# EvolvingLMMs-Lab/multimodal-sae

Measured on AMD Instinct MI355X. Metric: tokens/sec through SAE encode+TopK+decode, d=4096 width=131072, higher is better.
Workload: dtype int8 MFMA candidate select + f32 exact re-score/decode (outputs f32-exact); 1 GPU; BASELINE configs[1]: d_model=4096 width=131072 k=32, T=8192 bf16 activations/step resident in HBM, random-init unit-norm f32 weights; k=32, parallelism=single GPU, distinct_batches=4

## Files before the change

include/msae.h:

```cpp
#ifndef MSAE_H_
#define MSAE_H_

#include <stddef.h>
#include <stdint.h>

#ifdef __cplusplus
extern "C" {
#endif

#define MSAE_ABI_VERSION 4

enum { MSAE_F32 = 0, MSAE_BF16 = 1, MSAE_F16 = 2 };

enum {
  MSAE_EINVAL = -1,
  MSAE_EALIGN = -2,
  MSAE_EWS = -3,
  MSAE_ENOTIMPL = -4
};

enum { MSAE_COARSE_DEFAULT = -1, MSAE_COARSE_BF16 = 0, MSAE_COARSE_INT8 = 1, MSAE_COARSE_FP8 = 2 };
enum { MSAE_DITHER_DEFAULT = 0, MSAE_DITHER_ON = 1, MSAE_DITHER_OFF = 2 };
typedef struct msae_options {
  uint32_t size;
  int32_t coarse_mode;
  float guard_z;
  int32_t status_detail;
  void *profile;
  int32_t exact;
  int32_t dither;
  int32_t *rows_rescored;
  uint64_t dither_seed;
  int32_t certified;
  int32_t reserved2;
  const void *certified_operands;
} msae_options;
void msae_options_init(msae_options *opts);

int msae_abi_version(void);
const char *msae_error_string(int code);
const char *msae_target_arch(void);


int msae_pre_acts_f32(const void *x, int x_dtype, const float *W_enc, const float *b_enc,
                      const float *b_dec, int T, int d, int N, int relu, float *out, void *stream);

size_t msae_topk_ws_bytes(int T, int N, int k);
int msae_topk_f32(const float *latents, int T, int N, int k, float *vals, int32_t *idx, void *ws,
                  size_t ws_bytes, void *stream);


size_t msae_encoder_prepared_bytes(int N, int d);
int msae_encoder_prepare(const float *W_enc, int N, int d, void *prepared, void *stream);
int msae_encoder_prepare_opts(const float *W_enc, int N, int d, void *prepared, const msae_options *opts, void *stream);
size_t msae_encoder_certified_bytes(int N, int d);
int msae_encoder_prepare_certified(const float *W_enc, const float *b_enc, int N, int d, void *operands, void *stream);
int msae_encoder_refresh(const float *W_enc, int N, int d, void *prepared, const msae_options *opts,
                         void *stream);
int msae_encoder_refresh_for(const float *W_enc, int N, int d, void *prepared, int T_next, const msae_options *opts,
                             void *stream);

size_t msae_encode_topk_ws_bytes(int T, int d, int N, int k, const msae_options *opts);
int msae_encode_topk(const void *x, int x_dtype, const float *W_enc, const float *b_enc,
                     const float *b_dec, const void *prepared, int T, int d, int N, int k,
                     int set_feature, float set_value, int zero_feature, float *vals, int32_t *idx,
                     int32_t *status, void *ws, size_t ws_bytes, const msae_options *opts, void *stream);
int msae_encode_topk_i64(const void *x, int x_dtype, const float *W_enc, const float *b_enc,
                         const float *b_dec, const void *prepared, int T, int d, int N, int k,
                         int set_feature, float set_value, int zero_feature, float *vals, int64_t *idx,
                         int32_t *status, void *ws, size_t ws_bytes, const msae_options *opts, void *stream);

size_t msae_encode_topk_rows_ws_bytes(int max_rows, int N);
int msae_encode_topk_rows(const void *x, int x_dtype, const float *W_enc, const float *b_enc,
                          const float *b_dec, const int32_t *rows, const int32_t *n_rows, int max_rows,
                          int d, int N, int k, int set_feature, float set_value, int zero_feature,
                          float *vals, int64_t *idx, int32_t *status, void *ws, size_t ws_bytes, void *stream);

size_t msae_shard_record_bytes(int C);
int msae_shard_candidates(const void *x, int x_dtype, const float *b_enc_shard, const float *b_dec,
                          const void *prepared_shard, int T, int d, int N_shard, int k, int row_offset, int C,
                          int set_feature, int zero_feature, void *records, void *ws, size_t ws_bytes,
                          const msae_options *opts, void *stream);
size_t msae_rescore_candidates_ws_bytes(int T, int d, int N, int k, int G, int C);
int msae_rescore_candidates(const void *x, int x_dtype, const float *W_enc, const float *b_enc,
                            const float *b_dec, int T, int T_valid, int d, int N, int k, int G, int C,
                            const void *records, int set_feature, float set_value, int zero_feature,
                            float *vals, int64_t *idx, int32_t *status, void *ws, size_t ws_bytes,
                            const msae_options *opts, void *stream);


int msae_decode_f32(const int32_t *idx, const float *acts, const float *W_dec, const float *b_dec,
                    int A, int k, int N, int d, float *out, int32_t *status, void *stream);
int msae_decode_i64_f32(const int64_t *idx, const float *acts, const float *W_dec, const float *b_dec,
                        int A, int k, int N, int d, float *out, int32_t *status, void *stream);

int msae_decode_bwd_acts_f32(const int32_t *idx, const float *grad_out, const float *W_dec, int A,
                             int k, int N, int d, float *g_acts, int32_t *status, void *stream);

size_t msae_decode_bwd_wdec_ws_bytes(int A, int k, int N);
int msae_decode_bwd_wdec_f32(const int32_t *idx, const float *acts, const float *grad_out, int A,
                             int k, int N, int d, float *g_W_dec, float *row_sumsq, float *row_act_sum,
                             int32_t *status, void *ws, size_t ws_bytes, void *stream);

int msae_sparsify_count(const float *vals, const int32_t *idx, int B, int S, int k, float thresh,
                        const uint8_t *filter_bitmap, int N, int64_t *counts, void *stream);
int msae_sparsify_write(const float *vals, const int32_t *idx, int B, int S, int k, float thresh,
                        const uint8_t *filter_bitmap, int N, int64_t row_base,
                        const int64_t *counts, int64_t *locations, float *activations,
                        void *stream);

enum { MSAE_POOL_IMAGE = 0, MSAE_POOL_WINDOW = 1, MSAE_STATS_MAX_T = 65536 };
size_t msae_feature_stats_ws_bytes(int T, int k, int N);
int msae_feature_stats_update(const float *vals, const int32_t *idx, int B, int S, int k, float thresh, int N,
                              int mode, int pool_len, int window, int64_t row_base, int n_top, uint64_t *count,
                              float *act_max, double *act_sum, float *top_val, int64_t *top_id, void *ws,
                              size_t ws_bytes, void *stream);
int msae_feature_stats_merge(int N, int n_top, uint64_t *count, float *act_max, double *act_sum, float *top_val,
                             int64_t *top_id, const uint64_t *src_count, const float *src_max,
                             const double *src_sum, const float *src_val, const int64_t *src_id, void *stream);

typedef struct msae_feature_sample {
  uint32_t size;
  int32_t n_sample;
  uint64_t seed;
  uint64_t *seg_count;
  float *smp_val;
  int64_t *smp_id;
} msae_feature_sample;
int msae_feature_stats_update_sampled(const float *vals, const int32_t *idx, int B, int S, int k, float thresh, int N,
                                      int mode, int pool_len, int window, int64_t row_base, int n_top,
                                      uint64_t *count, float *act_max, double *act_sum, float *top_val,
                                      int64_t *top_id, const msae_feature_sample *sample, void *ws, size_t ws_bytes,
                                      void *stream);
int msae_feature_sample_merge(int N, int n_sample, uint64_t seed, uint64_t *seg_count, float *smp_val,
                              int64_t *smp_id, const uint64_t *src_seg_count, const float *src_val,
                              const int64_t *src_id, void *stream);

enum { MSAE_POOL_TOKEN = 2 };
enum { MSAE_COACT_JACCARD = 0, MSAE_COACT_COUNT = 1 };
size_t msae_coact_ws_bytes(int T, int k, int N);
int msae_coact_update(const float *vals, const int32_t *idx, int B, int S, int k, float thresh, int N, int mode,
                      int pool_len, int window, const int32_t *slot_of, int F, int32_t *counts, uint64_t *seg_count,
                      void *ws, size_t ws_bytes, void *stream);
int msae_coact_topk(const int32_t *counts, const int64_t *seg_count, const int32_t *queries, int F, int N, int m,
                    int metric, int exclude_self, float *out_val, int32_t *out_idx, void *stream);
int msae_coact_topk_i64(const int32_t *counts, const int64_t *seg_count, const int32_t *queries, int F, int N, int m,
                        int metric, int exclude_self, float *out_val, int64_t *out_idx, void *stream);

enum { MSAE_REDUCE_MEAN = 0, MSAE_REDUCE_MAX = 1, MSAE_PROBE_MAX_K = 256 };
int msae_pooled_acts_f32(const void *x, int x_dtype, const float *W_enc, const float *b_enc, const float *b_dec, int T,
                         int d, int N, const int32_t *seg, int S, const int32_t *chunks, int C, int reduce, float *out,
                         void *stream);
int msae_probe_maps_f32(const void *x, int x_dtype, const float *W_enc, const float *b_enc, const float *b_dec, int T,
                        int d, int N, const int32_t *seg, int S, const int32_t *idx, int k, float *maps, void *stream);

int msae_row_inv_norms_f32(const float *W, int N, int d, float *inv, void *stream);
size_t msae_rows_topk_ws_bytes(int M, int N, int k, int chunks);
int msae_rows_topk_f32(const float *Q, int Qn, const int32_t *q_rows, int M, const float *K, int N, int d,
                       const float *q_scale, const float *k_scale, const int32_t *exclude, int k, int chunks,
                       float *vals, int32_t *idx, void *ws, size_t ws_bytes, void *stream);
int msae_rows_topk_i64_f32(const float *Q, int Qn, const int32_t *q_rows, int M, const float *K, int N, int d,
                           const float *q_scale, const float *k_scale, const int32_t *exclude, int k, int chunks,
                           float *vals, int64_t *idx, void *ws, size_t ws_bytes, void *stream);

int msae_pre_acts_features_f32(const void *x, int x_dtype, const float *W_enc, const float *b_enc, const float *b_dec,
                               const int32_t *features, int M, int T, int d, int N, int relu,
                               float *out, int ld_out, void *stream);
int msae_topk_map_i64_f32(const float *latents, int T, int M, int k, int ld, const int32_t *col_map,
                          float *vals, int64_t *idx, void *stream);

enum { MSAE_EDIT_SET = 0, MSAE_EDIT_ZERO = 1 };
int msae_edit_topk_f32(const float *vals_in, const int32_t *idx_in, int T, int kk, const int32_t *edit_feat,
                       const float *edit_val, const int32_t *edit_kind, int E, int N, int k, float *vals, int32_t *idx,
                       void *stream);
int msae_edit_topk_i64_f32(const float *vals_in, const int64_t *idx_in, int T, int kk, const int32_t *edit_feat,
                           const float *edit_val, const int32_t *edit_kind, int E, int N, int k, float *vals,
                           int64_t *idx, void *stream);

int msae_edit_topk_rows_f32(const float *vals_in, const int32_t *idx_in, int T, int kk, const int32_t *group_of,
                            const int32_t *group_off, int G, const int32_t *edit_feat, const float *edit_val,
                            const int32_t *edit_kind, int E_total, int E_max, int N, int k, float *vals, int32_t *idx,
                            uint8_t *edited, void *stream);
int msae_edit_topk_rows_i64_f32(const float *vals_in, const int64_t *idx_in, int T, int kk, const int32_t *group_of,
                                const int32_t *group_off, int G, const int32_t *edit_feat, const float *edit_val,
                                const int32_t *edit_kind, int E_total, int E_max, int N, int k, float *vals, int64_t *idx,
                                uint8_t *edited, void *stream);

int msae_merge_topk(const int32_t *gathered, int T, int G, int kl, int k, float *vals, int32_t *idx,
                    int32_t *flagged, void *stream);
int msae_compact_flags(const int32_t *flags, int T, int32_t *rows, int32_t *n_rows, void *stream);
int msae_merge_topk_masked(const int32_t *gathered, int T, int G, int kl, int k, const int32_t *mask,
                           float *vals, int32_t *idx, int64_t *idx64, void *stream);

int msae_unit_norm_rows_f32(float *W, int N, int d, float eps, void *stream);
size_t msae_weighted_row_sum_ws_bytes(int N, int d);
int msae_weighted_row_sum_f32(const float *W, const float *s, int N, int d, float scale, float *out, void *ws,
                              size_t ws_bytes, void *stream);
int msae_sum_f32(const float *v, size_t n, float *accum, void *stream);
int msae_adam_rows_fused_f32(float *W, const float *G, float *M, float *V, int rows, int d,
                             const float *total_sumsq, float max_norm, int project, float lr, float beta1,
                             float beta2, float eps, int step, float renorm_eps, void *prepared, int T_next,
                             const msae_options *opts, void *stream);
int msae_grad_sumsq_f32(const float *g, size_t n, float *accum, void *stream);
int msae_adam_rows_f32(float *W, const float *G, float *M, float *V, int rows, int d,
                       const float *total_sumsq, float max_norm, int project, float lr, float beta1,
                       float beta2, float eps, int step, void *stream);

size_t msae_adam8_blocks(int rows, int d);
int msae_adam8_rows_f32(float *W, const float *G, uint8_t *M8, uint8_t *R8, float *SM, float *SR, int rows, int d,
                        const float *total_sumsq, float max_norm, int project, float lr, float beta1, float beta2,
                        float eps, int step, float renorm_eps, void *prepared, int T_next, const msae_options *opts,
                        void *stream);
int msae_adam8_quantize_f32(const float *M, const float *V, uint8_t *M8, uint8_t *R8, float *SM, float *SR, int rows,
                            int d, void *stream);
int msae_adam8_dequantize_f32(const uint8_t *M8, const uint8_t *R8, const float *SM, const float *SR, float *M, float *V,
                              int rows, int d, void *stream);

int msae_profile_create(int max_steps, void **handle);
int msae_profile_read(void *handle, float *stage_ms, int *n_steps);
int msae_profile_destroy(void *handle);

#ifdef __cplusplus
}
#endif
#endif
```

multimodal-sae_amd/csrc/capi.hip:

```cpp
#include "common.h"

extern "C" int msae_abi_version(void) { return MSAE_ABI_VERSION; }

extern "C" const char *msae_target_arch(void) { return "gfx950"; }

extern "C" const char *msae_error_string(int code) {
  switch (code) {
    case 0: return "success";
    case MSAE_EINVAL: return "msae: invalid argument (shape, k or dtype code)";
    case MSAE_EALIGN: return "msae: pointer or leading dimension not aligned as required";
    case MSAE_EWS: return "msae: workspace missing or too small";
    case MSAE_ENOTIMPL: return "msae: shape outside what this build supports";
    default: return code > 0 ? hipGetErrorString((hipError_t)code) : "msae: unknown error";
  }
}
```

multimodal-sae_amd/csrc/topk.hip:

```cpp
#include "common.h"
#include "sortsel.h"
#include "wave_ops.h"

namespace {

constexpr int TK_THREADS = 1024;
constexpr int TK_WAVES = TK_THREADS / 64;
constexpr int TK_BINS = 4096;

struct TkShared {
  unsigned hist[TK_BINS];
  unsigned wave_tot[TK_WAVES];
  unsigned bin;
  unsigned remaining;
  unsigned base_gt;
  unsigned base_eq;
};

template <bool VEC>
__device__ __forceinline__ void load4(const float *row, int i, int N, float (&v)[4]) {
  if constexpr (VEC) {
    f32x4 t = *reinterpret_cast<const f32x4 *>(row + i);
    v[0] = t[0]; v[1] = t[1]; v[2] = t[2]; v[3] = t[3];
  } else {
#pragma unroll
    for (int e = 0; e < 4; ++e) v[e] = (i + e < N) ? row[i + e] : 0.f;
  }
}

template <bool VEC>
__device__ __forceinline__ void radix_pass(const float *row, int N, unsigned prefix, unsigned mask,
                                           int shift, int nbins, TkShared &sh) {
  const unsigned need = sh.remaining;
  for (int b = threadIdx.x; b < nbins; b += TK_THREADS) sh.hist[b] = 0;
  __syncthreads();
  const int n4 = (N + 3) & ~3;
  for (int i = threadIdx.x * 4; i < n4; i += TK_THREADS * 4) {
    float v[4];
    load4<VEC>(row, i, N, v);
#pragma unroll
    for (int e = 0; e < 4; ++e) {
      if (VEC || i + e < N) {
        unsigned key = f32_order_key(v[e]);
        if ((key & mask) == prefix) atomicAdd(&sh.hist[(key >> shift) & (unsigned)(nbins - 1)], 1u);
      }
    }
  }
  __syncthreads();
  const int per = (nbins + TK_THREADS - 1) / TK_THREADS;
  const int rt = TK_THREADS - 1 - threadIdx.x;
  unsigned local = 0;
  for (int e = 0; e < per; ++e) {
    int b = nbins - 1 - (rt * per + e);
    if (b >= 0) local += sh.hist[b];
  }
  const int lane = threadIdx.x & 63, wave = threadIdx.x >> 6;
  unsigned incl = local;
#pragma unroll
  for (int off = 1; off < 64; off <<= 1) {
    unsigned n = __shfl_down(incl, off, 64);
    if (lane + off < 64) incl += n;
  }
  __syncthreads();
  if (lane == 0) sh.wave_tot[wave] = incl;
  __syncthreads();
  unsigned above = 0;
  for (int w = wave + 1; w < TK_WAVES; ++w) above += sh.wave_tot[w];
  above += incl - local;
  if (above < need && need <= above + local) {
    unsigned cum = above;
    for (int e = 0; e < per; ++e) {
      int b = nbins - 1 - (rt * per + e);
      if (b < 0) break;
      unsigned c = sh.hist[b];
      if (cum + c >= need) {
        sh.bin = (unsigned)b;
        sh.remaining = need - cum;
        break;
      }
      cum += c;
    }
  }
  __syncthreads();
}

template <bool VEC>
__global__ __launch_bounds__(TK_THREADS) void topk_rows_kernel(const float *__restrict__ latents,
                                                               int T, int N, int k, int ld,
                                                               const int *__restrict__ n_rows,
                                                               float *__restrict__ vals,
                                                               int32_t *__restrict__ idx, TopkExtra ex) {
  extern __shared__ __attribute__((aligned(16))) unsigned char smem_raw[];
  if (n_rows) T = min(T, *n_rows);
  TkShared &sh = *reinterpret_cast<TkShared *>(smem_raw);
  unsigned long long *keys = reinterpret_cast<unsigned long long *>(smem_raw + sizeof(TkShared));
  const int kp = next_pow2(k);
  for (int rowi = blockIdx.x; rowi < T; rowi += gridDim.x) {
  const float *row = latents + (size_t)rowi * ld;

  if (threadIdx.x == 0) {
    sh.remaining = (unsigned)k;
    sh.base_gt = 0;
    sh.base_eq = 0;
  }
  for (int i = threadIdx.x; i < kp; i += TK_THREADS) keys[i] = 0ull;
  __syncthreads();

  unsigned prefix = 0, mask = 0;
  radix_pass<VEC>(row, N, prefix, mask, 20, 4096, sh);
  prefix |= sh.bin << 20; mask |= 0xFFFu << 20;
  radix_pass<VEC>(row, N, prefix, mask, 8, 4096, sh);
  prefix |= sh.bin << 8; mask |= 0xFFFu << 8;
  radix_pass<VEC>(row, N, prefix, mask, 0, 256, sh);
  prefix |= sh.bin;
  const unsigned pivot = prefix;
  const unsigned r = sh.remaining;
  const unsigned n_gt = (unsigned)k - r;
  __syncthreads();

  const int n4 = (N + 3) & ~3;
  for (int base = 0; base < n4; base += TK_THREADS * 4) {
    const int i = base + threadIdx.x * 4;
    float v[4] = {0.f, 0.f, 0.f, 0.f};
    unsigned key[4];
    unsigned c_gt = 0, c_eq = 0;
    if (i < n4) load4<VEC>(row, i, N, v);
#pragma unroll
    for (int e = 0; e < 4; ++e) {
      const bool in = (i + e < N);
      key[e] = in ? f32_order_key(v[e]) : 0u;
      c_gt += (in && key[e] > pivot);
      c_eq += (in && key[e] == pivot);
    }
    const unsigned packed = c_gt | (c_eq << 16);
    if (__syncthreads_or((int)packed) == 0) continue;
    unsigned total;
    const unsigned ex = block_excl_scan<TK_WAVES>(packed, sh.wave_tot, &total);
    unsigned p_gt = sh.base_gt + (ex & 0xFFFFu);
    unsigned p_eq = sh.base_eq + (ex >> 16);
#pragma unroll
    for (int e = 0; e < 4; ++e) {
      if (i + e < N) {
        if (key[e] > pivot) {
          keys[p_gt++] = rank_key(v[e], i + e);
        } else if (key[e] == pivot) {
          if (p_eq < r) keys[n_gt + p_eq] = rank_key(v[e], i + e);
          ++p_eq;
        }
      }
    }
    __syncthreads();
    if (threadIdx.x == 0) {
      sh.base_gt += total & 0xFFFFu;
      sh.base_eq += total >> 16;
    }
    __syncthreads();
    if (sh.base_gt >= n_gt && sh.base_eq >= r) break;
  }
  __syncthreads();

  bitonic_sort_desc_u64<TK_THREADS>(keys, kp, threadIdx.x);
  const int orow = ex.row_map ? ex.row_map[rowi] : rowi;
  for (int j = threadIdx.x; j < k; j += TK_THREADS) {
    const unsigned long long kk = keys[j];
    const int ix = rank_key_index(kk);
    const int ox = ex.col_map ? ex.col_map[ix] : ix;
    if (idx) idx[(size_t)orow * k + j] = ox;
    if (ex.idx64) ex.idx64[(size_t)orow * k + j] = ox;
    vals[(size_t)orow * k + j] = row[ix];
  }
  if (ex.status && threadIdx.x == 0) ex.status[orow] = ex.detail ? (1 | ((ex.status[orow] & ~3) << 8)) : 1;
  __syncthreads();
  }
}

constexpr int KTH_LOW_BIT = 14;
template <int VPL>
__global__ __launch_bounds__(256) void kth_value_kernel(const float *__restrict__ rows, int T, int S,
                                                        int ld, int r, float *__restrict__ out,
                                                        int out_ld, int out_col, KthPush push) {
  const int lane = threadIdx.x & 63;
  const int t = blockIdx.x * 4 + (threadIdx.x >> 6);
  if (t >= T) return;
  const float *row = rows + (size_t)t * ld;
  unsigned key[VPL];
#pragma unroll
  for (int i = 0; i < VPL / 4; ++i) {
    const f32x4 v = *reinterpret_cast<const f32x4 *>(row + (i * 64 + lane) * 4);
    key[4 * i + 0] = f32_order_key(v[0]); key[4 * i + 1] = f32_order_key(v[1]);
    key[4 * i + 2] = f32_order_key(v[2]); key[4 * i + 3] = f32_order_key(v[3]);
  }
  unsigned lo = 0u;
  int first_bit = 31;
  {
    unsigned mx = 0u;
#pragma unroll
    for (int i = 0; i < VPL; ++i) mx = key[i] > mx ? key[i] : mx;
#pragma unroll
    for (int off = 32; off > 0; off >>= 1) { const unsigned o = __shfl_xor(mx, off, 64); mx = o > mx ? o : mx; }
    const unsigned pre = mx & 0xFF000000u;
    int c = 0;
#pragma unroll
    for (int i = 0; i < VPL; ++i) c += (key[i] >= pre) ? 1 : 0;
#pragma unroll
    for (int off = 32; off > 0; off >>= 1) c += __shfl_xor(c, off, 64);
    if (c >= r) { lo = pre; first_bit = 23; }
  }
#pragma unroll 1
  for (int bit = first_bit; bit >= KTH_LOW_BIT; --bit) {
    const unsigned mid = lo | (1u << bit);
    int c = 0;
#pragma unroll
    for (int i = 0; i < VPL; ++i) c += (key[i] >= mid) ? 1 : 0;
#pragma unroll
    for (int off = 32; off > 0; off >>= 1) c += __shfl_xor(c, off, 64);
    if (c >= r) lo = mid;
  }
  if (lane == 0) out[(size_t)t * out_ld + out_col] = f32_from_order_key(lo);
  if (push.cnt && f32_from_order_key(lo) > 0.f) {
    int total = 0;
#pragma unroll
    for (int i = 0; i < VPL; ++i) {
      total += __builtin_popcountll(__builtin_amdgcn_ballot_w64(key[i] > lo));
      if ((i & 7) == 7) asm volatile("" : "+s"(total));
    }
    if (total == 0) return;
    int base = 0;
    if (lane == 0) base = atomicAdd(push.cnt + (size_t)t * push.cnt_stride, total);
    base = __builtin_amdgcn_readfirstlane(base);
    unsigned long long *list = push.cand + (size_t)t * (push.row_stride ? push.row_stride : push.cap);
    unsigned lo2 = lo;
    asm volatile("" : "+v"(lo2));
#pragma unroll
    for (int i = 0; i < VPL; ++i) {
      const bool hit = key[i] > lo2;
      const unsigned long long m = __builtin_amdgcn_ballot_w64(hit);
      if (m == 0ull) continue;
      if (hit) {
        const int slot = base + (int)__builtin_amdgcn_mbcnt_hi((unsigned)(m >> 32), __builtin_amdgcn_mbcnt_lo((unsigned)m, 0u));
        const int j = ((i >> 2) * 64 + lane) * 4 + (i & 3);
        unsigned kk;
        asm volatile("v_mov_b32 %0, %1" : "=v"(kk) : "v"(key[i]));
        if (slot < push.cap) list[slot] = rank_key_from_order(kk, j * push.stride + push.off);
      }
      base += __builtin_popcountll(m);
      if ((i & 7) == 7) asm volatile("" : "+s"(base));
    }
  }
}

template <bool SECOND> struct MergeOut;
template <> struct MergeOut<false> { float *vals; int32_t *idx; int32_t *flagged; };
template <> struct MergeOut<true> { const int32_t *mask; float *vals; int32_t *idx; int64_t *idx64; };

template <bool SECOND>
__global__ __launch_bounds__(64) void merge_topk_kernel(const int32_t *__restrict__ gathered, int T, int G, int kl, int k,
                                                        MergeOut<SECOND> o) {
  extern __shared__ __attribute__((aligned(16))) unsigned long long mkeys[];
  const int lane = threadIdx.x, t = blockIdx.x;
  if constexpr (SECOND) { if (o.mask[t] == 0) return; }
  const int M = G * kl, np = next_pow2(M);
  unsigned long long worst_last = 0ull;
  for (int i = lane; i < np; i += 64) {
    unsigned long long key = 0ull;
    if (i < M) {
      const int g = i / kl, j = i % kl;
      const float v = __int_as_float(gathered[(((size_t)g * 2 + 0) * T + t) * kl + j]);
      const int f = gathered[(((size_t)g * 2 + 1) * T + t) * kl + j];
      key = rank_key(v, f);
      if constexpr (!SECOND) { if (j == kl - 1) worst_last = key > worst_last ? key : worst_last; }
    }
    mkeys[i] = key;
  }
  if constexpr (!SECOND) worst_last = wave_max(worst_last);
  bitonic_sort_desc_u64<64>(mkeys, np, lane);
  for (int j = lane; j < k; j += 64) {
    const unsigned long long key = mkeys[j];
    if constexpr (SECOND) {
      if (o.idx) o.idx[(size_t)t * k + j] = rank_key_index(key);
      if (o.idx64) o.idx64[(size_t)t * k + j] = rank_key_index(key);
    } else {
      o.idx[(size_t)t * k + j] = rank_key_index(key);
    }
    o.vals[(size_t)t * k + j] = rank_key_value(key);
  }
  if constexpr (!SECOND) { if (lane == 0 && o.flagged) o.flagged[t] = (kl < k && worst_last >= mkeys[k - 1]) ? 1 : 0; }
}

__global__ __launch_bounds__(1024) void compact_flags_kernel(const int32_t *__restrict__ flags, int T,
                                                             int32_t *__restrict__ rows, int32_t *__restrict__ n_rows) {
  __shared__ int wave_tot[16];
  const int lane = threadIdx.x & 63;
  int carry = 0;
  for (int base = 0; base < T; base += 1024) {
    const int t = base + threadIdx.x;
    const bool f = t < T && flags[t] != 0;
    const unsigned long long m = __builtin_amdgcn_ballot_w64(f);
    int total;
    const int off = carry + block_wave_offset<16>((int)__builtin_popcountll(m), wave_tot, &total);
    if (f) rows[off + __builtin_popcountll(m & ((1ull << lane) - 1ull))] = t;
    carry += total;
  }
  if (threadIdx.x == 0) *n_rows = carry;
}

}

extern "C" size_t msae_topk_ws_bytes(int T, int N, int k) {
  (void)T; (void)N; (void)k;
  return 0;
}

int msae_topk_launch(const float *latents, int T, int N, int k, int ld, const int *n_rows,
                     float *vals, int32_t *idx, hipStream_t s, const TopkExtra &ex) {
  if (T < 0 || N <= 0 || k <= 0 || k > N || k > 16384 || ld < N) return MSAE_EINVAL;
  if (T == 0) return 0;
  const size_t smem = sizeof(TkShared) + (size_t)next_pow2(k) * sizeof(unsigned long long);
  const bool vec = (N % 4 == 0) && (ld % 4 == 0) && msae_aligned(latents, 16);
  if (smem > 48 * 1024) {
    if (vec) MSAE_HIP_TRY(hipFuncSetAttribute((const void *)topk_rows_kernel<true>, hipFuncAttributeMaxDynamicSharedMemorySize, (int)smem));
    else MSAE_HIP_TRY(hipFuncSetAttribute((const void *)topk_rows_kernel<false>, hipFuncAttributeMaxDynamicSharedMemorySize, (int)smem));
  }
  const int grid = (n_rows && T > 128) ? 128 : T;
  if (vec)
    hipLaunchKernelGGL(topk_rows_kernel<true>, dim3(grid), dim3(TK_THREADS), smem, s, latents, T, N, k, ld,
                       n_rows, vals, idx, ex);
  else
    hipLaunchKernelGGL(topk_rows_kernel<false>, dim3(grid), dim3(TK_THREADS), smem, s, latents, T, N, k,
                       ld, n_rows, vals, idx, ex);
  return msae_launch_status();
}

bool msae_kth_value_launch(const float *rows, int T, int S, int ld, int r, float *out, int out_ld,
                           int out_col, hipStream_t s, const KthPush &push) {
  if (S % 256 || ld % 4 || !msae_aligned(rows, 16) || r < 1 || r > S) return false;
  const dim3 grid((T + 3) / 4), block(256);
  switch (S / 64) {
#define KTH_CASE(V) case V: hipLaunchKernelGGL(kth_value_kernel<V>, grid, block, 0, s, rows, T, S, ld, r, out, out_ld, out_col, push); return true;
    KTH_CASE(4) KTH_CASE(8) KTH_CASE(16) KTH_CASE(32) KTH_CASE(64) KTH_CASE(128)
#undef KTH_CASE
    default: return false;
  }
}

extern "C" int msae_topk_f32(const float *latents, int T, int N, int k, float *vals, int32_t *idx,
                             void *ws, size_t ws_bytes, void *stream) {
  (void)ws; (void)ws_bytes;
  return msae_topk_launch(latents, T, N, k, N, nullptr, vals, idx, (hipStream_t)stream, TopkExtra());
}

extern "C" int msae_topk_map_i64_f32(const float *latents, int T, int M, int k, int ld, const int32_t *col_map,
                                     float *vals, int64_t *idx, void *stream) {
  if (!latents || !col_map || !vals || !idx) return MSAE_EINVAL;
  TopkExtra ex;
  ex.idx64 = idx; ex.col_map = col_map;
  return msae_topk_launch(latents, T, M, k, ld, nullptr, vals, nullptr, (hipStream_t)stream, ex);
}

template <bool SECOND>
static int merge_topk_launch(const int32_t *gathered, int T, int G, int kl, int k, MergeOut<SECOND> o, void *stream) {
  if (T < 0 || G <= 0 || kl <= 0 || k <= 0 || (long)G * kl < k || (long)G * kl > 8192) return MSAE_EINVAL;
  if (T == 0) return 0;
  const size_t smem = (size_t)next_pow2(G * kl) * sizeof(unsigned long long);
  MSAE_HIP_TRY(hipFuncSetAttribute((const void *)merge_topk_kernel<SECOND>, hipFuncAttributeMaxDynamicSharedMemorySize, (int)smem));
  hipLaunchKernelGGL(merge_topk_kernel<SECOND>, dim3(T), dim3(64), smem, (hipStream_t)stream, gathered, T, G, kl, k, o);
  return msae_launch_status();
}

extern "C" int msae_merge_topk(const int32_t *gathered, int T, int G, int kl, int k, float *vals,
                               int32_t *idx, int32_t *flagged, void *stream) {
  return merge_topk_launch<false>(gathered, T, G, kl, k, {vals, idx, flagged}, stream);
}

extern "C" int msae_compact_flags(const int32_t *flags, int T, int32_t *rows, int32_t *n_rows, void *stream) {
  if (T < 0 || !rows || !n_rows || (T > 0 && !flags)) return MSAE_EINVAL;
  hipLaunchKernelGGL(compact_flags_kernel, dim3(1), dim3(1024), 0, (hipStream_t)stream, flags, T, rows, n_rows);
  return msae_launch_status();
}

extern "C" int msae_merge_topk_masked(const int32_t *gathered, int T, int G, int kl, int k, const int32_t *mask,
                                      float *vals, int32_t *idx, int64_t *idx64, void *stream) {
  if (!mask || !vals || (!idx && !idx64)) return MSAE_EINVAL;
  return merge_topk_launch<true>(gathered, T, G, kl, k, {mask, vals, idx, idx64}, stream);
}
```

multimodal-sae_amd/msae/_hip.py:

```python
from __future__ import annotations

import ctypes
import os
from pathlib import Path

import torch

_LIB_DIR = Path(__file__).resolve().parent / "_lib"
LIB_PATH = _LIB_DIR / "libmsae_hip.so"

c_void_p, c_int, c_float, c_size_t, c_int64 = (ctypes.c_void_p, ctypes.c_int, ctypes.c_float,
                                               ctypes.c_size_t, ctypes.c_int64)

ABI_VERSION = 4


class MsaeOptions(ctypes.Structure):
    _fields_ = [("size", ctypes.c_uint32), ("coarse_mode", ctypes.c_int32), ("guard_z", ctypes.c_float),
                ("status_detail", ctypes.c_int32), ("profile", ctypes.c_void_p), ("exact", ctypes.c_int32),
                ("dither", ctypes.c_int32), ("rows_rescored", ctypes.c_void_p), ("dither_seed", ctypes.c_uint64),
                ("certified", ctypes.c_int32), ("reserved2", ctypes.c_int32), ("certified_operands", ctypes.c_void_p)]


c_opts_p = ctypes.POINTER(MsaeOptions)


class MsaeFeatureSample(ctypes.Structure):
    _fields_ = [("size", ctypes.c_uint32), ("n_sample", ctypes.c_int32), ("seed", ctypes.c_uint64),
                ("seg_count", ctypes.c_void_p), ("smp_val", ctypes.c_void_p), ("smp_id", ctypes.c_void_p)]


c_sample_p = ctypes.POINTER(MsaeFeatureSample)

PROTOTYPES = {
    "msae_options_init": (None, [c_opts_p]),
    "msae_abi_version": (c_int, []),
    "msae_error_string": (ctypes.c_char_p, [c_int]),
    "msae_target_arch": (ctypes.c_char_p, []),
    "msae_pre_acts_f32": (c_int, [c_void_p, c_int, c_void_p, c_void_p, c_void_p, c_int, c_int, c_int,
                                  c_int, c_void_p, c_void_p]),
    "msae_topk_ws_bytes": (c_size_t, [c_int, c_int, c_int]),
    "msae_topk_f32": (c_int, [c_void_p, c_int, c_int, c_int, c_void_p, c_void_p, c_void_p, c_size_t,
                              c_void_p]),
    "msae_encoder_prepared_bytes": (c_size_t, [c_int, c_int]),
    "msae_encoder_prepare": (c_int, [c_void_p, c_int, c_int, c_void_p, c_void_p]),
    "msae_encoder_prepare_opts": (c_int, [c_void_p, c_int, c_int, c_void_p, c_opts_p, c_void_p]),
    "msae_encoder_certified_bytes": (c_size_t, [c_int, c_int]),
    "msae_encoder_prepare_certified": (c_int, [c_void_p, c_void_p, c_int, c_int, c_void_p, c_void_p]),
    "msae_encoder_refresh": (c_int, [c_void_p, c_int, c_int, c_void_p, c_opts_p, c_void_p]),
    "msae_encoder_refresh_for": (c_int, [c_void_p, c_int, c_int, c_void_p, c_int, c_opts_p, c_void_p]),
    "msae_encode_topk_ws_bytes": (c_size_t, [c_int, c_int, c_int, c_int, c_opts_p]),
    "msae_encode_topk": (c_int, [c_void_p, c_int, c_void_p, c_void_p, c_void_p, c_void_p, c_int, c_int,
                                 c_int, c_int, c_int, c_float, c_int, c_void_p, c_void_p, c_void_p,
                                 c_void_p, c_size_t, c_opts_p, c_void_p]),
    "msae_encode_topk_i64": (c_int, [c_void_p, c_int, c_void_p, c_void_p, c_void_p, c_void_p, c_int, c_int,
                                     c_int, c_int, c_int, c_float, c_int, c_void_p, c_void_p, c_void_p,
                                     c_void_p, c_size_t, c_opts_p, c_void_p]),
    "msae_encode_topk_rows_ws_bytes": (c_size_t, [c_int, c_int]),
    "msae_encode_topk_rows": (c_int, [c_void_p, c_int, c_void_p, c_void_p, c_void_p, c_void_p, c_void_p, c_int, c_int,
                                      c_int, c_int, c_int, c_float, c_int, c_void_p, c_void_p, c_void_p, c_void_p,
                                      c_size_t, c_void_p]),
    "msae_shard_record_bytes": (c_size_t, [c_int]),
    "msae_shard_candidates": (c_int, [c_void_p, c_int, c_void_p, c_void_p, c_void_p, c_int, c_int, c_int, c_int,
                                      c_int, c_int, c_int, c_int, c_void_p, c_void_p, c_size_t, c_opts_p, c_void_p]),
    "msae_rescore_candidates_ws_bytes": (c_size_t, [c_int, c_int, c_int, c_int, c_int, c_int]),
    "msae_rescore_candidates": (c_int, [c_void_p, c_int, c_void_p, c_void_p, c_void_p, c_int, c_int, c_int, c_int,
                                        c_int, c_int, c_int, c_void_p, c_int, c_float, c_int, c_void_p, c_void_p,
                                        c_void_p, c_void_p, c_size_t, c_opts_p, c_void_p]),
    "msae_decode_f32": (c_int, [c_void_p, c_void_p, c_void_p, c_void_p, c_int, c_int, c_int, c_int,
                                c_void_p, c_void_p, c_void_p]),
    "msae_decode_i64_f32": (c_int, [c_void_p, c_void_p, c_void_p, c_void_p, c_int, c_int, c_int, c_int,
                                    c_void_p, c_void_p, c_void_p]),
    "msae_decode_bwd_acts_f32": (c_int, [c_void_p, c_void_p, c_void_p, c_int, c_int, c_int, c_int,
                                         c_void_p, c_void_p, c_void_p]),
    "msae_decode_bwd_wdec_ws_bytes": (c_size_t, [c_int, c_int, c_int]),
    "msae_decode_bwd_wdec_f32": (c_int, [c_void_p, c_void_p, c_void_p, c_int, c_int, c_int, c_int,
                                         c_void_p, c_void_p, c_void_p, c_void_p, c_void_p, c_size_t, c_void_p]),
    "msae_sparsify_count": (c_int, [c_void_p, c_void_p, c_int, c_int, c_int, c_float, c_void_p, c_int,
                                    c_void_p, c_void_p]),
    "msae_sparsify_write": (c_int, [c_void_p, c_void_p, c_int, c_int, c_int, c_float, c_void_p, c_int,
                                    c_int64, c_void_p, c_void_p, c_void_p, c_void_p]),
    "msae_feature_stats_ws_bytes": (c_size_t, [c_int, c_int, c_int]),
    "msae_feature_stats_update": (c_int, [c_void_p, c_void_p, c_int, c_int, c_int, c_float, c_int, c_int, c_int, c_int,
                                          c_int64, c_int, c_void_p, c_void_p, c_void_p, c_void_p, c_void_p, c_void_p,
                                          c_size_t, c_void_p]),
    "msae_feature_stats_merge": (c_int, [c_int, c_int, c_void_p, c_void_p, c_void_p, c_void_p, c_void_p, c_void_p,
                                         c_void_p, c_void_p, c_void_p, c_void_p, c_void_p]),
    "msae_feature_stats_update_sampled": (c_int, [c_void_p, c_void_p, c_int, c_int, c_int, c_float, c_int, c_int, c_int,
                                                  c_int, c_int64, c_int, c_void_p, c_void_p, c_void_p, c_void_p, c_void_p,
                                                  c_sample_p, c_void_p, c_size_t, c_void_p]),
    "msae_feature_sample_merge": (c_int, [c_int, c_int, ctypes.c_uint64, c_void_p, c_void_p, c_void_p, c_void_p, c_void_p,
                                          c_void_p, c_void_p]),
    "msae_coact_ws_bytes": (c_size_t, [c_int, c_int, c_int]),
    "msae_coact_update": (c_int, [c_void_p, c_void_p, c_int, c_int, c_int, c_float, c_int, c_int, c_int, c_int, c_void_p,
                                  c_int, c_void_p, c_void_p, c_void_p, c_size_t, c_void_p]),
    "msae_coact_topk": (c_int, [c_void_p, c_void_p, c_void_p, c_int, c_int, c_int, c_int, c_int, c_void_p, c_void_p,
                                c_void_p]),
    "msae_coact_topk_i64": (c_int, [c_void_p, c_void_p, c_void_p, c_int, c_int, c_int, c_int, c_int, c_void_p, c_void_p,
                                    c_void_p]),
    "msae_pooled_acts_f32": (c_int, [c_void_p, c_int, c_void_p, c_void_p, c_void_p, c_int, c_int, c_int, c_void_p, c_int,
                                     c_void_p, c_int, c_int, c_void_p, c_void_p]),
    "msae_probe_maps_f32": (c_int, [c_void_p, c_int, c_void_p, c_void_p, c_void_p, c_int, c_int, c_int, c_void_p, c_int,
                                    c_void_p, c_int, c_void_p, c_void_p]),
    "msae_row_inv_norms_f32": (c_int, [c_void_p, c_int, c_int, c_void_p, c_void_p]),
    "msae_rows_topk_ws_bytes": (c_size_t, [c_int, c_int, c_int, c_int]),
    "msae_rows_topk_f32": (c_int, [c_void_p, c_int, c_void_p, c_int, c_void_p, c_int, c_int, c_void_p, c_void_p, c_void_p,
                                   c_int, c_int, c_void_p, c_void_p, c_void_p, c_size_t, c_void_p]),
    "msae_rows_topk_i64_f32": (c_int, [c_void_p, c_int, c_void_p, c_int, c_void_p, c_int, c_int, c_void_p, c_void_p, c_void_p,
                                       c_int, c_int, c_void_p, c_void_p, c_void_p, c_size_t, c_void_p]),
    "msae_pre_acts_features_f32": (c_int, [c_void_p, c_int, c_void_p, c_void_p, c_void_p, c_void_p, c_int, c_int, c_int,
                                           c_int, c_int, c_void_p, c_int, c_void_p]),
    "msae_topk_map_i64_f32": (c_int, [c_void_p, c_int, c_int, c_int, c_int, c_void_p, c_void_p, c_void_p, c_void_p]),
    "msae_edit_topk_f32": (c_int, [c_void_p, c_void_p, c_int, c_int, c_void_p, c_void_p, c_void_p, c_int, c_int, c_int,
                                   c_void_p, c_void_p, c_void_p]),
    "msae_edit_topk_i64_f32": (c_int, [c_void_p, c_void_p, c_int, c_int, c_void_p, c_void_p, c_void_p, c_int, c_int, c_int,
                                       c_void_p, c_void_p, c_void_p]),
    "msae_edit_topk_rows_f32": (c_int, [c_void_p, c_void_p, c_int, c_int, c_void_p, c_void_p, c_int, c_void_p, c_void_p,
                                        c_void_p, c_int, c_int, c_int, c_int, c_void_p, c_void_p, c_void_p, c_void_p]),
    "msae_edit_topk_rows_i64_f32": (c_int, [c_void_p, c_void_p, c_int, c_int, c_void_p, c_void_p, c_int, c_void_p, c_void_p,
                                            c_void_p, c_int, c_int, c_int, c_int, c_void_p, c_void_p, c_void_p, c_void_p]),
    "msae_merge_topk": (c_int, [c_void_p, c_int, c_int, c_int, c_int, c_void_p, c_void_p, c_void_p, c_void_p]),
    "msae_compact_flags": (c_int, [c_void_p, c_int, c_void_p, c_void_p, c_void_p]),
    "msae_merge_topk_masked": (c_int, [c_void_p, c_int, c_int, c_int, c_int, c_void_p, c_void_p, c_void_p, c_void_p,
                                       c_void_p]),
    "msae_unit_norm_rows_f32": (c_int, [c_void_p, c_int, c_int, c_float, c_void_p]),
    "msae_grad_sumsq_f32": (c_int, [c_void_p, c_size_t, c_void_p, c_void_p]),
    "msae_sum_f32": (c_int, [c_void_p, c_size_t, c_void_p, c_void_p]),
    "msae_weighted_row_sum_ws_bytes": (c_size_t, [c_int, c_int]),
    "msae_weighted_row_sum_f32": (c_int, [c_void_p, c_void_p, c_int, c_int, c_float, c_void_p, c_void_p, c_size_t, c_void_p]),
    "msae_adam_rows_fused_f32": (c_int, [c_void_p, c_void_p, c_void_p, c_void_p, c_int, c_int, c_void_p, c_float,
                                         c_int, c_float, c_float, c_float, c_float, c_int, c_float, c_void_p, c_int,
                                         c_opts_p, c_void_p]),
    "msae_adam_rows_f32": (c_int, [c_void_p, c_void_p, c_void_p, c_void_p, c_int, c_int, c_void_p, c_float,
                                   c_int, c_float, c_float, c_float, c_float, c_int, c_void_p]),
    "msae_adam8_blocks": (c_size_t, [c_int, c_int]),
    "msae_adam8_rows_f32": (c_int, [c_void_p, c_void_p, c_void_p, c_void_p, c_void_p, c_void_p, c_int, c_int, c_void_p,
                                    c_float, c_int, c_float, c_float, c_float, c_float, c_int, c_float, c_void_p, c_int,
                                    c_opts_p, c_void_p]),
    "msae_adam8_quantize_f32": (c_int, [c_void_p, c_void_p, c_void_p, c_void_p, c_void_p, c_void_p, c_int, c_int, c_void_p]),
    "msae_adam8_dequantize_f32": (c_int, [c_void_p, c_void_p, c_void_p, c_void_p, c_void_p, c_void_p, c_int, c_int,
                                          c_void_p]),
    "msae_profile_create": (c_int, [c_int, ctypes.POINTER(c_void_p)]),
    "msae_profile_read": (c_int, [c_void_p, c_void_p, c_void_p]),
    "msae_profile_destroy": (c_int, [c_void_p]),
}

DTYPE_CODE = {torch.float32: 0, torch.bfloat16: 1, torch.float16: 2}

_lib = None


class MsaeLibraryMissing(RuntimeError):
    pass


def load() -> ctypes.CDLL:
    global _lib
    if _lib is not None:
        return _lib
    path = Path(os.environ.get("MSAE_HIP_LIB", LIB_PATH))
    if not path.exists():
        raise MsaeLibraryMissing(
            f"{path} not found: build it with `python __graft_entry__.py` "
            "(multimodal-sae_amd/csrc/build.sh). There is no CPU fallback for the SAE kernels.")
    lib = ctypes.CDLL(str(path))
    for name, (res, args) in PROTOTYPES.items():
        fn = getattr(lib, name)
        fn.restype, fn.argtypes = res, args
    if lib.msae_abi_version() != ABI_VERSION:
        raise RuntimeError(f"libmsae_hip.so ABI version {lib.msae_abi_version()} != {ABI_VERSION}: rebuild it "
                           "(python __graft_entry__.py)")
    _lib = lib
    return lib


class MsaeNotImplemented(RuntimeError):
    """MSAE_ENOTIMPL: the shape lies outside what this entry point supports (callers with an alternative take it)."""


def check(code: int, what: str) -> None:
    if code != 0:
        msg = load().msae_error_string(code).decode()
        raise (MsaeNotImplemented if code == -4 else RuntimeError)(f"{what} failed: {msg} (code {code})")


def ptr(t: torch.Tensor | None):
    if t is None:
        return None
    return c_void_p(t.data_ptr())


def stream_of(t: torch.Tensor):
    return c_void_p(torch.cuda.current_stream(t.device).cuda_stream)


def require_device(*tensors: torch.Tensor | None) -> torch.device:
    dev = None
    for t in tensors:
        if t is None:
            continue
        if not t.is_cuda:
            raise RuntimeError(
                "msae kernels run on MI355X only: got a tensor on "
                f"{t.device}. Move the Sae and its inputs to a HIP device (there is no CPU path).")
        if dev is None:
            dev = t.device
        elif t.device != dev:
            raise RuntimeError(f"tensors on different devices: {dev} vs {t.device}")
    return dev
```

Before: 1.553 million tokens/s.

## Add streaming kth-value kernel with first-chunk threshold and LDS candidate buffer

After: 1.576 million tokens/s, median of 6. 1.01x the previous value.

```diff
diff --git a/include/msae.h b/include/msae.h
--- a/include/msae.h
+++ b/include/msae.h
@@ -192,6 +192,9 @@
 int msae_merge_topk_masked(const int32_t *gathered, int T, int G, int kl, int k, const int32_t *mask,
                            float *vals, int32_t *idx, int64_t *idx64, void *stream);
 
+int msae_kth_value_f32(const float *rows, int T, int S, int ld, int r, float *out, int32_t *cnt,
+                       unsigned long long *cand, int cap, int stride, int off, void *stream);
+
 int msae_unit_norm_rows_f32(float *W, int N, int d, float eps, void *stream);
 size_t msae_weighted_row_sum_ws_bytes(int N, int d);
 int msae_weighted_row_sum_f32(const float *W, const float *s, int N, int d, float scale, float *out, void *ws,
diff --git a/multimodal-sae_amd/csrc/capi.hip b/multimodal-sae_amd/csrc/capi.hip
--- a/multimodal-sae_amd/csrc/capi.hip
+++ b/multimodal-sae_amd/csrc/capi.hip
@@ -14,3 +14,17 @@
     default: return code > 0 ? hipGetErrorString((hipError_t)code) : "msae: unknown error";
   }
 }
+
+bool msae_kth_value_launch(const float *rows, int T, int S, int ld, int r, float *out, int out_ld, int out_col, hipStream_t s,
+                           const KthPush &push);
+
+extern "C" int msae_kth_value_f32(const float *rows, int T, int S, int ld, int r, float *out, int32_t *cnt,
+                                  unsigned long long *cand, int cap, int stride, int off, void *stream) {
+  if (!rows || !out || T < 0 || S <= 0 || ld < S || r < 1 || r > S || (cnt && (!cand || cap < 0 || stride < 1 || off < 0)))
+    return MSAE_EINVAL;
+  if (T == 0) return 0;
+  KthPush push{};
+  if (cnt) { push.cnt = cnt; push.cand = cand; push.cap = cap; push.stride = stride; push.off = off; }
+  if (!msae_kth_value_launch(rows, T, S, ld, r, out, 1, 0, (hipStream_t)stream, push)) return MSAE_ENOTIMPL;
+  return msae_launch_status();
+}
diff --git a/multimodal-sae_amd/csrc/topk.hip b/multimodal-sae_amd/csrc/topk.hip
--- a/multimodal-sae_amd/csrc/topk.hip
+++ b/multimodal-sae_amd/csrc/topk.hip
@@ -1,3 +1,5 @@
+#include <stdlib.h>
+
 #include "common.h"
 #include "sortsel.h"
 #include "wave_ops.h"
@@ -245,6 +247,151 @@
       }
       base += __builtin_popcountll(m);
       if ((i & 7) == 7) asm volatile("" : "+s"(base));
+    }
+  }
+}
+
+constexpr int KS_CHUNK = 1024, KS_CAP = 512;
+
+__device__ __forceinline__ int wave_count(bool p) { return (int)__builtin_popcountll(__builtin_amdgcn_ballot_w64(p)); }
+__device__ __forceinline__ int lanes_below(unsigned long long m) {
+  return (int)__builtin_amdgcn_mbcnt_hi((unsigned)(m >> 32), __builtin_amdgcn_mbcnt_lo((unsigned)m, 0u));
+}
+__device__ __forceinline__ int kth_push_reserve(const KthPush &push, int t, int lane, int total) {
+  int base = 0;
+  if (lane == 0) base = atomicAdd(push.cnt + (size_t)t * push.cnt_stride, total);
+  return __builtin_amdgcn_readfirstlane(base);
+}
+
+__global__ __launch_bounds__(256, 8) void kth_stream_kernel(const float *__restrict__ rows, int T, int S, int ld, int r,
+                                                            float *__restrict__ out, int out_ld, int out_col, KthPush push) {
+  __shared__ unsigned s_key[4][KS_CAP];
+  __shared__ int s_col[4][KS_CAP];
+  const int lane = threadIdx.x & 63, w = threadIdx.x >> 6;
+  const int t = blockIdx.x * 4 + w;
+  if (t >= T) return;
+  const float *row = rows + (size_t)t * ld;
+  unsigned *sk = s_key[w];
+  int *sc = s_col[w];
+  const int nchunk = S / KS_CHUNK;
+  f32x4 nxt[4];
+#pragma unroll
+  for (int q = 0; q < 4; ++q) nxt[q] = *reinterpret_cast<const f32x4 *>(row + (q * 64 + lane) * 4);
+  unsigned lo0 = 0u;
+  int n = 0;
+#pragma unroll 1
+  for (int c = 0; c < nchunk && n <= KS_CAP; ++c) {
+    unsigned key[16];
+#pragma unroll
+    for (int q = 0; q < 4; ++q) {
+      key[4 * q + 0] = f32_order_key(nxt[q][0]); key[4 * q + 1] = f32_order_key(nxt[q][1]);
+      key[4 * q + 2] = f32_order_key(nxt[q][2]); key[4 * q + 3] = f32_order_key(nxt[q][3]);
+    }
+    if (c + 1 < nchunk) {
+#pragma unroll
+      for (int q = 0; q < 4; ++q) nxt[q] = *reinterpret_cast<const f32x4 *>(row + (c + 1) * KS_CHUNK + (q * 64 + lane) * 4);
+    }
+    if (c == 0) {
+#pragma unroll 1
+      for (int bit = 31; bit >= KTH_LOW_BIT; --bit) {
+        const unsigned mid = lo0 | (1u << bit);
+        int cnt = 0;
+#pragma unroll
+        for (int i = 0; i < 16; ++i) cnt += wave_count(key[i] >= mid);
+        if (cnt >= r) lo0 = mid;
+      }
+    }
+#pragma unroll
+    for (int i = 0; i < 16; ++i) {
+      const bool hit = key[i] >= lo0;
+      const unsigned long long m = __builtin_amdgcn_ballot_w64(hit);
+      if (m == 0ull) continue;
+      const int slot = n + lanes_below(m);
+      if (hit && slot < KS_CAP) {
+        sk[slot] = key[i];
+        sc[slot] = c * KS_CHUNK + ((i >> 2) * 64 + lane) * 4 + (i & 3);
+      }
+      n += (int)__builtin_popcountll(m);
+    }
+  }
+  const bool pushing = push.cnt != nullptr;
+  unsigned long long *list = pushing ? push.cand + (size_t)t * (push.row_stride ? push.row_stride : push.cap) : nullptr;
+  unsigned lo = 0u;
+  if (n <= KS_CAP) {
+    __builtin_amdgcn_fence(__ATOMIC_RELEASE, "wavefront");
+    __builtin_amdgcn_wave_barrier();
+    __builtin_amdgcn_fence(__ATOMIC_ACQUIRE, "wavefront");
+    unsigned k8[KS_CAP / 64];
+#pragma unroll
+    for (int i = 0; i < KS_CAP / 64; ++i) k8[i] = (i * 64 + lane < n) ? sk[i * 64 + lane] : 0u;
+#pragma unroll 1
+    for (int bit = 31; bit >= KTH_LOW_BIT; --bit) {
+      const unsigned mid = lo | (1u << bit);
+      bool take = mid <= lo0;
+      if (!take) {
+        int cnt = 0;
+#pragma unroll
+        for (int i = 0; i < KS_CAP / 64; ++i) cnt += wave_count(k8[i] >= mid);
+        take = cnt >= r;
+      }
+      if (take) lo = mid;
+    }
+    if (lane == 0) out[(size_t)t * out_ld + out_col] = f32_from_order_key(lo);
+    if (!pushing || !(f32_from_order_key(lo) > 0.f)) return;
+    int total = 0;
+#pragma unroll
+    for (int i = 0; i < KS_CAP / 64; ++i) total += wave_count(k8[i] > lo);
+    if (total == 0) return;
+    int base = kth_push_reserve(push, t, lane, total);
+#pragma unroll
+    for (int i = 0; i < KS_CAP / 64; ++i) {
+      const bool hit = k8[i] > lo;
+      const unsigned long long m = __builtin_amdgcn_ballot_w64(hit);
+      if (m == 0ull) continue;
+      const int slot = base + lanes_below(m);
+      if (hit && slot < push.cap) list[slot] = rank_key_from_order(k8[i], sc[i * 64 + lane] * push.stride + push.off);
+      base += (int)__builtin_popcountll(m);
+    }
+    return;
+  }
+#pragma unroll 1
+  for (int bit = 31; bit >= KTH_LOW_BIT; --bit) {
+    const unsigned mid = lo | (1u << bit);
+    bool take = mid <= lo0;
+    if (!take) {
+      int cnt = 0;
+#pragma unroll 1
+      for (int j = lane * 4; j < S; j += 256) {
+        const f32x4 v = *reinterpret_cast<const f32x4 *>(row + j);
+        cnt += (f32_order_key(v[0]) >= mid) + (f32_order_key(v[1]) >= mid) + (f32_order_key(v[2]) >= mid) + (f32_order_key(v[3]) >= mid);
+      }
+      take = wave_sum(cnt) >= r;
+    }
+    if (take) lo = mid;
+  }
+  if (lane == 0) out[(size_t)t * out_ld + out_col] = f32_from_order_key(lo);
+  if (!pushing || !(f32_from_order_key(lo) > 0.f)) return;
+  int total = 0;
+#pragma unroll 1
+  for (int j = lane * 4; j < S; j += 256) {
+    const f32x4 v = *reinterpret_cast<const f32x4 *>(row + j);
+    total += (f32_order_key(v[0]) > lo) + (f32_order_key(v[1]) > lo) + (f32_order_key(v[2]) > lo) + (f32_order_key(v[3]) > lo);
+  }
+  total = wave_sum(total);
+  if (total == 0) return;
+  int base = kth_push_reserve(push, t, lane, total);
+#pragma unroll 1
+  for (int j = lane * 4; j < S; j += 256) {
+    const f32x4 v = *reinterpret_cast<const f32x4 *>(row + j);
+#pragma unroll
+    for (int e = 0; e < 4; ++e) {
+      const unsigned key = f32_order_key(v[e]);
+      const bool hit = key > lo;
+      const unsigned long long m = __builtin_amdgcn_ballot_w64(hit);
+      if (m == 0ull) continue;
+      const int slot = base + lanes_below(m);
+      if (hit && slot < push.cap) list[slot] = rank_key_from_order(key, (j + e) * push.stride + push.off);
+      base += (int)__builtin_popcountll(m);
     }
   }
 }
@@ -335,6 +482,11 @@
                            int out_col, hipStream_t s, const KthPush &push) {
   if (S % 256 || ld % 4 || !msae_aligned(rows, 16) || r < 1 || r > S) return false;
   const dim3 grid((T + 3) / 4), block(256);
+  const char *e = getenv("MSAE_KTH_STREAM");
+  if (S % KS_CHUNK == 0 && S >= 2 * KS_CHUNK && (long)r * (S / KS_CHUNK) <= KS_CAP / 2 && !(e && e[0] == '0')) {
+    hipLaunchKernelGGL(kth_stream_kernel, grid, block, 0, s, rows, T, S, ld, r, out, out_ld, out_col, push);
+    return true;
+  }
   switch (S / 64) {
 #define KTH_CASE(V) case V: hipLaunchKernelGGL(kth_value_kernel<V>, grid, block, 0, s, rows, T, S, ld, r, out, out_ld, out_col, push); return true;
     KTH_CASE(4) KTH_CASE(8) KTH_CASE(16) KTH_CASE(32) KTH_CASE(64) KTH_CASE(128)
diff --git a/multimodal-sae_amd/msae/_hip.py b/multimodal-sae_amd/msae/_hip.py
--- a/multimodal-sae_amd/msae/_hip.py
+++ b/multimodal-sae_amd/msae/_hip.py
@@ -123,6 +123,8 @@
     "msae_compact_flags": (c_int, [c_void_p, c_int, c_void_p, c_void_p, c_void_p]),
     "msae_merge_topk_masked": (c_int, [c_void_p, c_int, c_int, c_int, c_int, c_void_p, c_void_p, c_void_p, c_void_p,
                                        c_void_p]),
+    "msae_kth_value_f32": (c_int, [c_void_p, c_int, c_int, c_int, c_int, c_void_p, c_void_p, c_void_p, c_int, c_int, c_int,
+                                   c_void_p]),
     "msae_unit_norm_rows_f32": (c_int, [c_void_p, c_int, c_int, c_float, c_void_p]),
     "msae_grad_sumsq_f32": (c_int, [c_void_p, c_size_t, c_void_p, c_void_p]),
     "msae_sum_f32": (c_int, [c_void_p, c_size_t, c_void_p, c_void_p]),
```
